# heitorrapela/HalluciDet

Measured on AMD Instinct MI355X. Metric: images/sec train_hallucidet (640x512, batch 8/GPU), higher is better.
Workload: dtype f16; 1 GPU; train_hallucidet.py fasterrcnn LLVIP batch=8 fp16 on 1xMI355X (BASELINE configs[1]); U-Net resnet34 fwd+bwd, 3 frozen Faster R-CNN R50-FPN passes @300x300 (one batched evaluation of 24 images: trunk, RPN, RoI heads, NMS for all three; the RGB / IR passes' LOSS VALUES, which the reference computes and discards, are not evaluated), loss scaling, value clip 0.5, Adam; global_batch=8, image=1x512x640 IR + 3x512x640 RGB, batch_per_gpu=8, parallelism=dp1

## Files before the change

### hallucidet_amd/_abi.py

```python
import ctypes as C
import os

_HERE = os.path.dirname(os.path.abspath(__file__))
LIB_PATH = os.environ.get("HD_HIP_LIB") or os.path.join(_HERE, "lib", "libhallucidet_hip.so")

ABI_VERSION = 6

HD_ACT_NONE, HD_ACT_RELU, HD_ACT_SIGMOID = 0, 1, 2
HD_OUT_NHWC_F16, HD_OUT_NCHW_F32, HD_OUT_NHWC_F32 = 0, 1, 2

c_i32 = C.c_int32
c_i64 = C.c_int64
c_f = C.c_float
c_d = C.c_double
vp = C.c_void_p


class HipLibraryMissing(RuntimeError):
    pass


class HipCallError(RuntimeError):
    pass


class ConvArgs(C.Structure):
    _fields_ = [
        ("x", vp), ("x2", vp), ("w", vp), ("bias", vp), ("res", vp), ("mask", vp), ("y", vp), ("stats", vp),
        ("N", c_i32), ("Hsrc", c_i32), ("Wsrc", c_i32), ("Hin", c_i32), ("Win", c_i32),
        ("C1", c_i32), ("C2", c_i32), ("Ho", c_i32), ("Wo", c_i32), ("Cout", c_i32),
        ("KH", c_i32), ("KW", c_i32), ("stride", c_i32), ("pad", c_i32),
        ("up1", c_i32), ("in_dil", c_i32), ("act", c_i32), ("out_mode", c_i32),
        ("in_scale", vp), ("in_shift", vp), ("in_relu", c_i32), ("out_pool2", c_i32),
        ("bs_y", vp), ("bs_z", vp), ("bs_mean", vp), ("bs_invstd", vp), ("bs_gamma", vp), ("bs_beta", vp), ("bs_relu", c_i32), ("reserved1", c_i32),
        ("y2", vp),
    ]


class WprepDesc(C.Structure):
    _fields_ = [("w_oihw", C.c_void_p), ("w_fwd", C.c_void_p), ("w_dgrad", C.c_void_p)] + \
               [(n, C.c_int32) for n in ("Cout", "Cin", "KH", "KW", "Cin_pad", "Cout_pad")]


class WredDesc(C.Structure):
    _fields_ = [("slab", C.c_void_p), ("dw_oihw", C.c_void_p)] + \
               [(n, C.c_int32) for n in ("nsplit", "Cout_slab", "Cout", "KH", "KW", "Cin", "Cin_real", "accumulate")] + \
               [("scale", C.c_float)] + [(n, C.c_int32) for n in ("mode", "first_block", "reserved")]


class WgradArgs(C.Structure):
    _fields_ = [
        ("x", vp), ("x2", vp), ("dy", vp), ("slab", vp),
        ("N", c_i32), ("Hsrc", c_i32), ("Wsrc", c_i32), ("Hin", c_i32), ("Win", c_i32),
        ("C1", c_i32), ("C2", c_i32), ("Ho", c_i32), ("Wo", c_i32), ("Cout", c_i32),
        ("KH", c_i32), ("KW", c_i32), ("stride", c_i32), ("pad", c_i32), ("up1", c_i32),
        ("nsplit", c_i32),
        ("in_scale", vp), ("in_shift", vp), ("in_relu", c_i32), ("reserved0", c_i32),
        ("dw_oihw", vp), ("dw_scale", c_f), ("reserved1", c_i32),
    ]


PROTOTYPES = {
    "hd_abi_version": (C.c_int, []),
    "hd_last_error": (C.c_char_p, []),
    "hd_arch": (C.c_char_p, []),
    "hd_conv2d": (C.c_int, [C.POINTER(ConvArgs), vp]),
    "hd_conv2d_stats_rows": (C.c_int, [C.POINTER(ConvArgs)]),
    "hd_conv2d_pool2_ok": (C.c_int, [C.POINTER(ConvArgs)]),
    "hd_conv2d_bstat_ok": (C.c_int, [C.POINTER(ConvArgs)]),
    "hd_conv7x7s2_dgrad_thin": (C.c_int, [vp, vp, vp, vp] + [C.c_int] * 5 + [vp]),
    "hd_conv_tune_override": (C.c_int, [C.c_int] * 4),
    "hd_conv_tune_w8": (C.c_int, [C.c_int, C.c_int]),
    "hd_conv_nominal_batch": (C.c_int, [C.c_int]),
    "hd_gemm_w8_mode": (C.c_int, [C.c_int]),
    "hd_wgrad_w8_blocks": (C.c_int, [C.POINTER(WgradArgs)]),
    "hd_wgrad": (C.c_int, [C.POINTER(WgradArgs), vp]),
    "hd_wgrad_multi": (C.c_int, [C.POINTER(WgradArgs), C.c_int, vp]),
    "hd_wgrad_direct_ok": (C.c_int, [C.POINTER(WgradArgs)]),
    "hd_conv2d_wgrad": (C.c_int, [C.POINTER(ConvArgs), C.POINTER(WgradArgs), vp]),
    "hd_conv2d_multi": (C.c_int, [C.POINTER(ConvArgs), C.c_int, vp]),
    "hd_wgrad_tune_override": (C.c_int, [C.c_int]),
    "hd_wgrad_reduce": (C.c_int, [vp, vp] + [C.c_int] * 7 + [c_f, C.c_int, vp]),
    "hd_wgrad_reduce_plan": (C.c_int, [vp, C.c_int]),
    "hd_wgrad_reduce_multi": (C.c_int, [vp, C.c_int, C.c_int, vp]),
    "hd_weight_prep": (C.c_int, [vp, vp, vp, vp] + [C.c_int] * 6 + [vp]),
    "hd_weight_prep_multi": (C.c_int, [vp, C.c_int, C.c_int, vp]),
    "hd_colsum": (C.c_int, [vp, C.c_int, C.c_int, vp, vp, vp]),
    "hd_rowsum": (C.c_int, [vp, C.c_int, C.c_int, vp, C.c_int, vp]),
    "hd_bn_finalize": (C.c_int, [vp, C.c_int, C.c_int, c_d, vp, vp, vp, vp, c_f, c_f, vp, vp, vp, vp, vp]),
    "hd_bn_eval_scale_shift": (C.c_int, [vp, vp, vp, vp, c_f, C.c_int, vp, vp, vp]),
    "hd_bn_apply": (C.c_int, [vp, vp, vp, vp, vp, c_i64, C.c_int, C.c_int, vp]),
    "hd_bn_bwd_reduce": (C.c_int, [vp] * 8 + [C.c_int, c_i64, C.c_int, C.c_int, vp]),
    "hd_bn_bwd_apply": (C.c_int, [vp] * 8 + [C.c_int] + [vp] * 5 + [c_f, C.c_int, c_i64, C.c_int, C.c_int, vp]),
    "hd_maxpool3x3s2": (C.c_int, [vp, vp] + [C.c_int] * 6 + [vp]),
    "hd_maxpool3x3s2_bwd": (C.c_int, [vp, vp, vp] + [C.c_int] * 6 + [vp]),
    "hd_maxpool3x3s2_idx": (C.c_int, [vp, vp, vp] + [C.c_int] * 6 + [vp]),
    "hd_maxpool3x3s2_bwd_idx": (C.c_int, [vp, vp, vp] + [C.c_int] * 6 + [vp]),
    "hd_maxpool3x3s2_bwd_idx_add": (C.c_int, [vp, vp, vp, vp] + [C.c_int] * 6 + [vp]),
    "hd_concat_up_bwd": (C.c_int, [vp, vp, vp] + [C.c_int] * 5 + [vp]),
    "hd_subsample2": (C.c_int, [vp, vp] + [C.c_int] * 6 + [vp]),
    "hd_subsample2_bwd": (C.c_int, [vp, vp] + [C.c_int] * 7 + [vp]),
    "hd_nchw_to_nhwc_resize": (C.c_int, [vp, vp] + [C.c_int] * 7 + [vp]),
    "hd_nchw_to_nhwc_resize_strided": (C.c_int, [vp, c_i64, c_i64, vp] + [C.c_int] * 7 + [vp]),
    "hd_nchw_to_nhwc_resize_bwd": (C.c_int, [vp, vp] + [C.c_int] * 7 + [c_f, vp]),
    "hd_nhwc_to_nchw": (C.c_int, [vp, vp] + [C.c_int] * 5 + [vp]),
    "hd_upsample_add": (C.c_int, [vp, vp, vp] + [C.c_int] * 6 + [vp]),
    "hd_upsample_add_bwd": (C.c_int, [vp, vp] + [C.c_int] * 7 + [vp]),
    "hd_upsample2_bwd": (C.c_int, [vp, vp] + [C.c_int] * 7 + [vp]),
    "hd_add_f16": (C.c_int, [vp, vp, vp, c_i64, vp]),
    "hd_slice_channels": (C.c_int, [vp, vp, c_i64, C.c_int, C.c_int, C.c_int, C.c_int, vp]),
    "hd_sigmoid_bwd_nchw_to_nhwc": (C.c_int, [vp, vp, vp] + [C.c_int] * 5 + [c_f, vp]),
    "hd_relu_bwd": (C.c_int, [vp, vp, vp, c_i64, vp]),
    "hd_f32_to_f16": (C.c_int, [vp, vp, c_i64, c_f, vp]),
    "hd_f16_to_f32": (C.c_int, [vp, vp, c_i64, c_f, vp]),
    "hd_pad_cast_f32_f16": (C.c_int, [vp, vp, C.c_int64, C.c_int, C.c_int, C.c_int64, C.c_int64, vp]),
    "hd_pad_cast_f32_f16_multi": (C.c_int, [vp, vp, vp, vp, vp, vp, vp, C.c_int, vp]),
    "hd_channel_sum_f16": (C.c_int, [vp, c_i64, C.c_int, vp, C.c_int, vp]),
    "hd_scale_store": (C.c_int, [vp, vp, C.c_int, c_f, C.c_int, vp]),
    "hd_nms_sorted_batched": (C.c_int, [vp, vp, C.c_int, C.c_int, c_f, vp, vp, vp]),
    "hd_nms_sorted_batched_topk": (C.c_int, [vp, vp, C.c_int, C.c_int, c_f, vp, vp, C.c_int, vp]),
    "hd_roi_align": (C.c_int, [vp, vp, vp] + [C.c_int] * 7 + [c_f, C.c_int, vp]),
    "hd_roi_align_ml": (C.c_int, [vp, vp, vp, vp, C.c_int, vp, vp, vp] + [C.c_int] * 5 + [vp]),
    "hd_roi_align_ml_bwd": (C.c_int, [vp, vp, vp, vp, vp, vp, vp] + [C.c_int] * 6 + [vp]),
    "hd_roi_align_ml_bwd_gather": (C.c_int, [vp, vp, vp, vp, vp, vp, vp] + [C.c_int] * 7 + [vp]),
    "hd_roi_align_bwd": (C.c_int, [vp, vp, vp] + [C.c_int] * 7 + [c_f, C.c_int, vp]),
    "hd_box_iou": (C.c_int, [vp, C.c_int, vp, C.c_int, vp, vp]),
    "hd_box_iou_batched": (C.c_int, [vp, C.c_int, vp, C.c_int, C.c_int, C.c_int, vp, vp]),
    "hd_rpn_loss": (C.c_int, [vp, vp, vp, vp, vp, vp, C.c_int64, C.c_float, vp, C.c_float, vp, vp, vp]),
    "hd_rpn_loss_bwd": (C.c_int, [vp, vp, vp, vp, vp, vp, C.c_int64, C.c_float, vp, vp, vp, C.c_float, vp, vp, vp]),
    "hd_retinanet_loss": (C.c_int, [vp] * 6 + [C.c_int] * 4 + [C.c_float] * 3 + [vp, vp, vp, vp, vp]),
    "hd_retinanet_loss_bwd": (C.c_int, [vp] * 6 + [C.c_int] * 4 + [C.c_float] * 3 + [vp] * 7),
    "hd_sigmoid_focal_loss": (C.c_int, [vp, vp, C.c_int64, C.c_float, C.c_float, vp, vp, vp]),
    "hd_groupnorm8_relu": (C.c_int, [vp] * 5 + [C.c_int] * 3 + [C.c_float, C.c_int, vp]),
    "hd_groupnorm8_relu_bwd": (C.c_int, [vp] * 6 + [C.c_int] * 4 + [vp]),
    "hd_groupnorm8_param_grad": (C.c_int, [vp] * 6 + [C.c_int] * 4 + [C.c_float, C.c_int, vp]),
    "hd_fcos_match": (C.c_int, [vp] * 3 + [C.c_int] * 5 + [C.c_float, vp, vp]),
    "hd_fcos_loss": (C.c_int, [vp] * 7 + [C.c_int] * 4 + [C.c_float] * 2 + [vp] * 4),
    "hd_fcos_loss_bwd": (C.c_int, [vp] * 7 + [C.c_int] * 4 + [C.c_float] * 2 + [vp] * 6),
    "hd_fastrcnn_loss": (C.c_int, [vp, vp, vp, vp, C.c_int, C.c_int, C.c_float, vp, vp, vp]),
    "hd_fastrcnn_loss_bwd": (C.c_int, [vp, vp, vp, vp, C.c_int, C.c_int, C.c_float, vp, vp, vp, vp, vp]),
    "hd_fastrcnn_loss_masked": (C.c_int, [vp, vp, vp, vp, C.c_int, C.c_int, C.c_float, vp, vp, vp, vp]),
    "hd_fastrcnn_loss_masked_bwd": (C.c_int, [vp, vp, vp, vp, C.c_int, C.c_int, C.c_float, vp, vp, vp, vp, vp, vp]),
    "hd_pixel_loss": (C.c_int, [vp, vp, vp] + [C.c_int] * 5 + [c_f, c_f, C.c_int] + [vp] * 6),
    "hd_map_match": (C.c_int, [vp] * 4 + [C.c_int] * 2 + [vp] * 3 + [C.c_int, vp, C.c_int] + [vp] * 9),
    "hd_map_accumulate": (C.c_int, [vp, vp, vp, c_i64, vp, vp, C.c_int, vp, vp, vp, vp]),
    "hd_sample_pos_neg": (C.c_int, [vp, vp, C.c_int, C.c_int, C.c_int, C.c_int, vp, vp, vp, vp]),
    "hd_roi_postprocess": (C.c_int, [vp, vp, vp, C.c_long, vp, C.c_int, C.c_int, C.c_int, vp] + [C.c_float] * 5 + [vp] * 4),
    "hd_roi_samples_padded": (C.c_int, [vp] * 7 + [C.c_int] * 4 + [vp] * 6),
    "hd_roi_samples_finish": (C.c_int, [vp, C.c_int, vp, vp, vp, vp, vp, C.c_int, C.c_int, vp, vp, vp, vp, vp]),
    "hd_roi_levels": (C.c_int, [vp, C.c_long, C.c_int, C.c_float, C.c_float, C.c_float, C.c_int, C.c_int, vp, vp]),
    "hd_batched_nms_pick": (C.c_int, [vp, vp, vp, vp, C.c_int, C.c_int, C.c_float, C.c_int, vp, vp, vp, vp, vp, vp, vp]),
    "hd_batched_nms_pick_segments": (C.c_int, [vp, vp, vp, C.c_int, C.c_int, vp, C.c_int, C.c_float, C.c_int, vp, vp, vp, vp, vp, vp, vp, vp, vp, vp]),
    "hd_rpn_decode_filter": (C.c_int, [vp, vp, vp, vp, C.c_int, C.c_int, C.c_int, C.c_float, C.c_float, C.c_float, C.c_float, C.c_float, vp, vp, vp, vp]),
    "hd_roi_decode_clip": (C.c_int, [vp, vp, C.c_long, C.c_int, C.c_int, vp, C.c_float, C.c_float, C.c_float, vp, vp]),
    "hd_topk_select_rows": (C.c_int, [vp, C.c_int, C.c_long, vp, C.c_int, C.c_int, vp, C.c_long, vp]),
    "hd_match_targets": (C.c_int, [vp, vp, vp, C.c_int, vp, C.c_int, C.c_int, C.c_int, C.c_float, C.c_float, C.c_int, vp, vp, vp, vp, vp, vp]),
    "hd_adam_step": (C.c_int, [vp, vp, vp, vp, c_i64] + [c_f] * 9 + [vp, vp]),
# ... 64 lines not shown
```

### hallucidet_amd/csrc/conv_dispatch.hip

```cpp
#include <stdlib.h>

#include "conv_params.h"

namespace {

int pick_bn(int Cout) { return Cout > 64 ? 128 : (Cout > 32 ? 64 : 32); }
int pick_bm(int M, int Cout) {
  int bn = pick_bn(Cout);
  int64_t blocks128 = (int64_t)hd_cdiv(M, 128) * hd_cdiv(Cout, bn);
  return (bn > 32 && blocks128 < 512) ? 64 : 128;
}

int fill_params(const hd_conv_args* a, ConvP& p) {
  HD_CHECK_ARG(a && a->x && a->w && a->y, "hd_conv2d: null pointer");
  HD_CHECK_ARG(a->C1 > 0 && a->C1 % 8 == 0 && a->C2 >= 0 && a->C2 % 8 == 0, "hd_conv2d: channel counts must be multiples of 8 (C1=%d C2=%d)", a->C1, a->C2);
  HD_CHECK_ARG((a->C2 == 0) == (a->x2 == nullptr), "hd_conv2d: x2/C2 mismatch");
  HD_CHECK_ARG(a->N > 0 && a->Ho > 0 && a->Wo > 0 && a->Cout > 0 && a->KH > 0 && a->KW > 0 && a->stride > 0, "hd_conv2d: bad extent");
  HD_CHECK_ARG(!(a->in_dil > 1 && (a->up1 || a->C2)), "hd_conv2d: in_dil excludes up1/x2");
  HD_CHECK_ARG(a->in_dil <= 2, "hd_conv2d: in_dil must be 1 or 2 (strides on the hot path)");
  HD_CHECK_ARG(a->C2 == 0 || (a->C1 % 32 == 0 && a->C2 % 32 == 0), "hd_conv2d: dual-source gather needs C1, C2 multiples of 32 (a K tile holds channels of one source)");
  HD_CHECK_ARG(!a->up1 || (a->Hin == 2 * a->Hsrc && a->Win == 2 * a->Wsrc), "hd_conv2d: up1 needs Hin=2*Hsrc");
  HD_CHECK_ARG((int64_t)a->N * a->Ho * a->Wo < (1ll << 31), "hd_conv2d: too many pixels");
  p.x = (const f16*)a->x;
  p.x2 = (const f16*)a->x2;
  p.w = (const f16*)a->w;
  p.bias = a->bias;
  p.res = (const f16*)a->res;
  p.mask = (const f16*)a->mask;
  p.y = a->y;
  p.stats = a->stats;
  p.N = a->N; p.Hsrc = a->Hsrc; p.Wsrc = a->Wsrc; p.Hin = a->Hin; p.Win = a->Win;
  p.C1 = a->C1; p.C2 = a->C2; p.Cin = a->C1 + a->C2;
  p.Ho = a->Ho; p.Wo = a->Wo; p.Cout = a->Cout; p.KH = a->KH; p.KW = a->KW;
  p.stride = a->stride; p.pad = a->pad; p.up1 = a->up1; p.in_dil = a->in_dil < 1 ? 1 : a->in_dil;
  p.act = a->act; p.out_mode = a->out_mode;
  HD_CHECK_ARG((a->in_scale == nullptr) == (a->in_shift == nullptr), "hd_conv2d: in_scale / in_shift must be given together");
  p.in_scale = a->in_scale; p.in_shift = a->in_shift; p.in_relu = a->in_relu;
  p.pool2 = a->out_pool2;
  p.y2 = a->y2;
  p.bs_y = (const f16*)a->bs_y; p.bs_z = (const f16*)a->bs_z;
  p.bs_mean = a->bs_mean; p.bs_invstd = a->bs_invstd; p.bs_gamma = a->bs_gamma; p.bs_beta = a->bs_beta; p.bs_relu = a->bs_relu;
  HD_CHECK_ARG(!p.bs_y || (p.stats && p.bs_mean && p.bs_invstd && !a->mask && a->act == HD_ACT_NONE && a->out_mode == HD_OUT_NHWC_F16 && !a->bias),
               "hd_conv2d: bs_* (BatchNorm backward sums) need stats, bs_mean, bs_invstd and exclude mask / act / bias / non-f16 output");
  HD_CHECK_ARG(p.out_mode >= HD_OUT_NHWC_F16 && p.out_mode <= HD_OUT_NHWC_F32, "hd_conv2d: out_mode %d", p.out_mode);
  p.M = a->N * a->Ho * a->Wo;
  p.cin8 = p.Cin / 8;
  p.nchunks = a->KH * a->KW * p.cin8;
  p.nk = 0;
  p.Ktot = a->KH * a->KW * p.Cin;
  p.prio = 0;
  p.par = p.ph = p.pw = p.Hc = p.Wc = p.t0h = p.t0w = 0;
  p.gm = p.gn = 0;
  p.tgroup = 1;
  p.inv_cin8 = 1.0f / (float)p.cin8;
  p.inv_kw = 1.0f / (float)a->KW;
  int64_t xb = (int64_t)a->N * a->Hsrc * a->Wsrc * a->C1 * 2;
  int64_t x2b = a->x2 ? (int64_t)a->N * a->Hin * a->Win * a->C2 * 2 : 0;
  int64_t wb = (int64_t)a->Cout * p.Ktot * 2;
  HD_CHECK_ARG(xb < 0xFFFFFFF0ll && x2b < 0xFFFFFFF0ll && wb < 0xFFFFFFF0ll, "hd_conv2d: tensor larger than 4 GiB (buffer addressing)");
  p.xbytes = (unsigned)xb; p.x2bytes = (unsigned)x2b; p.wbytes = (unsigned)wb;
  return HD_OK;
}

int env_int(const char* name, int dflt) {
  const char* v = getenv(name);
  return v ? atoi(v) : dflt;
}

}

static bool g_small_ok = true;

bool use_small(const ConvP& p) {
  static const int on = env_int("HD_CONV_SMALL", 1);
  return on && g_small_ok && hd_conv_small_eligible(p);
}

bool use_c64(const ConvP& p) {
  static const int on = env_int("HD_CONV_C64", 1);
  return on && g_small_ok && hd_conv_c64_eligible(p);
}

bool use_stem(const ConvP& p) {
  static const int on = env_int("HD_CONV_STEM", 1);
  return on && g_small_ok && hd_conv_stem_eligible(p);
}

bool use_c32(const ConvP& p) {
  static const int on = env_int("HD_CONV_C32", 1);
  return on && g_small_ok && !p.stats && hd_conv_c32to128_eligible(p);
}

bool use_cat(const ConvP& p) {
  static const int on = env_int("HD_CONV_CAT", 1);
  return on && g_small_ok && hd_conv_cat128to32_eligible(p);
}

static int g_gemm8_mode = -1;
extern "C" int hd_gemm_w8_mode(int mode) {
  HD_CHECK_ARG(mode == -1 || mode == 0 || mode == 128 || mode == 1128, "hd_gemm_w8_mode: mode in {-1, 0, 128, 1128}");
  g_gemm8_mode = mode;
  return HD_OK;
}
bool hd_gemm_w8_eligible(const ConvP& p);
void hd_gemm_w8_launch(ConvP& p, int tile, hipStream_t s);
static int choose_gemm8(const ConvP& p) {
  static const int on = env_int("HD_GEMM8", 1);
  if (!on || g_gemm8_mode == 0 || !g_small_ok || !hd_gemm_w8_eligible(p)) return 0;
  if (g_gemm8_mode > 0) return g_gemm8_mode;
  if (p.res || p.M < 2048 || p.Cout < 512 || p.Ktot < 512) return 0;
  const int64_t t128 = (int64_t)hd_cdiv(p.M, 256) * hd_cdiv(p.Cout, 128), t1128 = (int64_t)hd_cdiv(p.M, 128) * hd_cdiv(p.Cout, 128);
  if (t128 >= 160 && t128 <= 256) return 128;
  if (t1128 >= 200) return 1128;
  return 0;
}

static int g_ov_bm = -1, g_ov_bn = -1, g_ov_bk = -1, g_ov_deep = -1;
extern "C" int hd_conv_tune_override(int bm, int bn, int bk, int deep) {
  HD_CHECK_ARG((bm == -1 || bm == 64 || bm == 128) && (bn == -1 || bn == 32 || bn == 64 || bn == 128) && (bk == -1 || bk == 32 || bk == 64) &&
               deep >= -1 && deep <= 1, "hd_conv_tune_override: bm in {64,128}, bn in {32,64,128}, bk in {32,64}, deep in {0,1} or -1");
  g_ov_bm = bm; g_ov_bn = bn; g_ov_bk = bk; g_ov_deep = deep;
  g_small_ok = (bm == -1 && bn == -1 && bk == -1 && deep == -1);
  return HD_OK;
}

#ifdef HD_CONV_TRACE
static unsigned long long* g_trace = nullptr;
extern "C" int hd_conv_trace_buffer(void* buf) {
  g_trace = (unsigned long long*)buf;
  return HD_OK;
}
#endif

static int g_nominal_batch = 0;
extern "C" int hd_conv_nominal_batch(int n) {
  HD_CHECK_ARG(n >= 0 && n <= 4096, "hd_conv_nominal_batch: n in [0, 4096]");
  g_nominal_batch = n;
  return HD_OK;
}

static int choose_p8(const ConvP& p, bool allow_m160 = true) {
  static const int on = env_int("HD_CONV_P8", 1);
  if (!on || !hd_conv_p8_eligible(p)) return -1;
  if (p.Cout < 128 && !p.x2) return -1;
  static const int th[4] = {32, 16, 32, 16}, bn[4] = {128, 128, 64, 64};
  static const int ts = env_int("HD_W8_TS", 1);
  static const double step_ss[4] = {1270., 790., 800., 540.}, step_ts[4] = {1270., 790., 860., 450.}, fixed[4] = {11500., 8000., 9000., 7000.};
  double step[4];
  for (int c = 0; c < 4; ++c) step[c] = ((ts >= 2 && c >= 1) || (ts == 1 && c == 3)) ? step_ts[c] : step_ss[c];
  const int nk = p.nchunks / 8;
  int best = -1;
  double best_t = 1e30;
  static const int nominal = env_int("HD_CONV_NOMINAL_BATCH", 0);
  const int nominal_batch = g_nominal_batch > 0 ? g_nominal_batch : (nominal > 0 ? nominal : p.N);
  for (int c = 0; c < 4; ++c) {
    if (bn[c] == 128 && p.Cout <= 64) continue;
    const int64_t tm = (int64_t)nominal_batch * hd_cdiv(p.Ho, th[c]) * hd_cdiv(p.Wo, 8);
    const double eff = (double)((int64_t)nominal_batch * p.Ho * p.Wo) / (double)(tm * th[c] * 8);
    if (eff < 0.7) continue;
    const int64_t blocks = tm * hd_cdiv(p.Cout, bn[c]);
    const double t = (double)hd_cdiv(blocks, 256) * (fixed[c] + nk * step[c])   ;
    if (t < best_t) {
      best_t = t;
      best = c;
    }
  }
  best = ((ts >= 2 && best >= 1) || (ts == 1 && best == 3)) ? best + 4 : best;
  static const int m160_on = env_int("HD_CONV_M160", 1);
  static const double m160_fixed[2] = {(double)env_int("HD_M160_FIXED", 9000), (double)env_int("HD_M320_FIXED", 10500)};
  static const double m160_step[2] = {(double)env_int("HD_M160_STEP", 460), (double)env_int("HD_M320_STEP", 790)};
  if (m160_on && allow_m160 && hd_conv_m160_eligible(p)) {
    if (best < 0) {
      const int64_t b64 = (int64_t)hd_cdiv((int64_t)nominal_batch * p.Ho * p.Wo, 64) * hd_cdiv(p.Cout, 64);
      best_t = (double)hd_cdiv(b64, 512) * (4000. + nk * 900.);
    }
    static const double m96_fixed[2] = {(double)env_int("HD_M96_FIXED", 6600), (double)env_int("HD_M96_FIXED2", 11000)};
    static const double m96_step[2] = {(double)env_int("HD_M96_STEP", 350), (double)env_int("HD_M96_STEP2", 420)};
    static const int m96_on = env_int("HD_CONV_M96", 1);
    for (int v = 0; v < 3; ++v) {
      if (v == 2 && (!m96_on || p.x2)) continue;
      const int th_ = v == 1 ? 8 : 4, tw_ = v == 2 ? 24 : 40;
      const int64_t tm = (int64_t)nominal_batch * hd_cdiv(p.Ho, th_) * hd_cdiv(p.Wo, tw_);
      const int64_t blocks = tm * hd_cdiv(p.Cout, 64);
      double t;
      if (v == 2) {
        const int pair = blocks > 256;
        t = (double)(pair ? hd_cdiv(blocks, 512) : 1) * (m96_fixed[pair] + nk * m96_step[pair]);
      } else {
        t = (double)hd_cdiv(blocks, 256) * (m160_fixed[v] + nk * m160_step[v]);
      }
      if (t < best_t) {
        best_t = t;
        best = 8 + v;
      }
    }
  }
  return best;
// ... 154 lines not shown
  if (ok) {
    mp.n = n;
    const bool launched = c0.use64 ? hd_conv_launch_bk64_multi(mp, c0.bm, c0.bn, c0.deep, (hipStream_t)stream)
                                   : hd_conv_launch_bk32_multi(mp, c0.bm, c0.bn, c0.deep, (hipStream_t)stream);
    if (launched) {
      HD_CHECK_LAUNCH();
      return HD_OK;
    }
  }
  static const int m96_multi_on = env_int("HD_CONV_M96_MULTI", 1);
  bool taken[HD_CONV_MULTI_MAX] = {};
  if (multi_on && m96_multi_on && n >= 2 && n <= HD_CONV_MULTI_MAX && g_small_ok && g_w8_cfg < 0) {
    static ConvMulti m96;
    m96.n = 0;
    for (int i = 0; i < n; ++i) {
      ConvP& p = m96.p[m96.n];
      int rc = fill_params(&args[i], p);
      if (rc) return rc;
      if (use_small(p) || use_c64(p) || use_stem(p) || use_c32(p) || use_cat(p) || choose_gemm8(p) || p.pool2 || p.x2) continue;
      if (choose_tile(p).p8cfg != 10) continue;
      HD_CHECK_ARG(!p.bs_y || bstat_kernel(p), "hd_conv2d_multi: bs_* on a problem whose kernel does not implement them");
#ifdef HD_CONV_TRACE
      p.trace = nullptr;
      p.trace_tid = 0;
#endif
      taken[i] = true;
      ++m96.n;
    }
    if (m96.n >= 2) {
      hd_conv_launch_m96_multi(m96, (hipStream_t)stream);
      HD_CHECK_LAUNCH();
    } else {
      for (int i = 0; i < n; ++i) taken[i] = false;
    }
  }
  for (int i = 0; i < n; ++i) {
    if (taken[i]) continue;
    int rc = hd_conv2d(&args[i], stream);
    if (rc) return rc;
  }
  return HD_OK;
}

extern "C" int hd_conv2d(const hd_conv_args* a, void* stream) {
  ConvP p;
  int rc = fill_params(a, p);
  if (rc) return rc;
  hipStream_t s = (hipStream_t)stream;
#ifdef HD_CONV_TRACE
  p.trace = g_trace;
  p.trace_tid = env_int("HD_TRACE_TID", 0);
#endif
  HD_CHECK_ARG(!p.bs_y || bstat_kernel(p), "hd_conv2d: bs_* (BatchNorm backward sums) are implemented by the 8-wave and the 64-channel 3x3 kernels only; "
                                           "ask hd_conv2d_bstat_ok first");
  HD_CHECK_ARG(!p.pool2 || pool2_kernel(p),
               "hd_conv2d: out_pool2 is implemented by the small-channel 3x3 kernel (all channels pooled), the 32 -> 128 channel kernel "
               "(64 pooled channels + y2) and the 8-wave 3x3 family (pooled channels a multiple of 128); ask hd_conv2d_pool2_ok first");
  if (use_small(p)) {
    hd_conv_launch_small(p, s);
    HD_CHECK_LAUNCH();
    return HD_OK;
  }
  if (use_c64(p)) {
    hd_conv_launch_c64(p, s);
    HD_CHECK_LAUNCH();
    return HD_OK;
  }
  if (use_stem(p)) {
    hd_conv_launch_stem(p, s);
    HD_CHECK_LAUNCH();
    return HD_OK;
  }
  if (use_c32(p)) {
    hd_conv_launch_c32to128(p, s);
    HD_CHECK_LAUNCH();
    return HD_OK;
  }
  if (use_cat(p)) {
    hd_conv_launch_cat128to32(p, s);
    HD_CHECK_LAUNCH();
    return HD_OK;
  }
  if (const int g8 = choose_gemm8(p)) {
    hd_gemm_w8_launch(p, g8, s);
    HD_CHECK_LAUNCH();
    return HD_OK;
  }
  HD_CHECK_ARG(!p.in_scale, "hd_conv2d: consumer-side BatchNorm (in_scale / in_shift) is implemented by the small-channel 3x3 kernel only "
                            "(3x3 / stride 1 / pad 1, one source, C1 in {8,16,32}, Cout in {16,32} or a <= 16-channel fp32 head)");
  static const int par_on = env_int("HD_CONV_PARITY", 1);
  const bool par = par_on && p.in_dil == 2 && !p.stats && p.stride == 1 && (p.cin8 % 4) == 0 && p.out_mode == HD_OUT_NHWC_F16 && g_small_ok &&
                   g_w8_cfg < 0;
  const int M_full = p.M;
  if (par) p.M = p.N * ((p.Ho + 1) / 2) * ((p.Wo + 1) / 2);
  const TileChoice c = choose_tile(p);
  static const int w8_prio = env_int("HD_W8_PRIO", 0);
  p.prio = w8_prio;
  const int bm = c.bm, bn = c.bn;
  const bool use64 = c.use64, deep = c.deep;
  if (par && c.p8cfg < 0 && (c.use64 ? (p.cin8 % 8) == 0 : true)) {
    p.par = 1;
  } else {
    p.M = M_full;
  }
  if (c.p8cfg >= 8) {
    hd_conv_launch_m160(p, c.p8cfg == 9 ? 8 : 4, c.p8cfg == 10 ? 24 : 40, s);
  } else if (c.p8cfg >= 0) {
    hd_conv_launch_p8(p, c.p8cfg, s);
  } else if (use64) hd_conv_launch_bk64(p, bm, bn, deep, s);
  else hd_conv_launch_bk32(p, bm, bn, deep, s);
  HD_CHECK_LAUNCH();
  return HD_OK;
}
```

### include/hallucidet_hip.h

```cpp
#ifndef HALLUCIDET_HIP_H
#define HALLUCIDET_HIP_H

#include <stdint.h>

#ifdef __cplusplus
extern "C" {
#endif

#define HD_OK 0
#define HD_E_ARG (-1)
#define HD_E_LAUNCH (-2)
#define HD_E_UNSUPPORTED (-3)

#define HD_ACT_NONE 0
#define HD_ACT_RELU 1
#define HD_ACT_SIGMOID 2

#define HD_OUT_NHWC_F16 0
#define HD_OUT_NCHW_F32 1
#define HD_OUT_NHWC_F32 2

int hd_abi_version(void);
const char* hd_last_error(void);
const char* hd_arch(void);

typedef struct hd_conv_args {
  const void* x;
  const void* x2;
  const void* w;
  const float* bias;
  const void* res;
  const void* mask;
  void* y;
  float* stats;
  int32_t N, Hsrc, Wsrc;
  int32_t Hin, Win;
  int32_t C1, C2;
  int32_t Ho, Wo, Cout;
  int32_t KH, KW, stride, pad;
  int32_t up1, in_dil;
  int32_t act, out_mode;
  const float* in_scale;
  const float* in_shift;
  int32_t in_relu;
  int32_t out_pool2;
  const void* bs_y;
  const void* bs_z;
  const float* bs_mean;
  const float* bs_invstd;
  const float* bs_gamma;
  const float* bs_beta;
  int32_t bs_relu, reserved1;
  void* y2;
} hd_conv_args;

int hd_conv2d(const hd_conv_args* a, void* stream);
int hd_conv2d_bstat_ok(const hd_conv_args* a);
int hd_conv2d_pool2_ok(const hd_conv_args* a);
int hd_conv2d_stats_rows(const hd_conv_args* a);
int hd_conv7x7s2_dgrad_thin(const void* dy, const void* mask_z, const void* w16, void* dx, int N, int Hl, int Wl, int H, int W, void* stream);
int hd_conv_tune_override(int bm, int bn, int bk, int deep);
int hd_conv_tune_w8(int cfg, int nslices);
int hd_conv_nominal_batch(int n);
int hd_gemm_w8_mode(int mode);

typedef struct hd_wgrad_args {
  const void* x;
  const void* x2;
  const void* dy;
  float* slab;
  int32_t N, Hsrc, Wsrc, Hin, Win, C1, C2, Ho, Wo, Cout;
  int32_t KH, KW, stride, pad, up1;
  int32_t nsplit;
  const float* in_scale;
  const float* in_shift;
  int32_t in_relu, reserved0;
  float* dw_oihw;
  float dw_scale;
  int32_t reserved1;
} hd_wgrad_args;
int hd_wgrad(const hd_wgrad_args* a, void* stream);
int hd_wgrad_direct_ok(const hd_wgrad_args* a);
#define HD_WGRAD_MULTI_MAX 24
int hd_wgrad_multi(const hd_wgrad_args* args, int n, void* stream);
int hd_wgrad_w8_blocks(const hd_wgrad_args* a);
int hd_wgrad_tune_override(int tm);
int hd_conv2d_multi(const hd_conv_args* args, int n, void* stream);

int hd_conv2d_wgrad(const hd_conv_args* dgrad, const hd_wgrad_args* wgrad, void* stream);

int hd_wgrad_reduce(const float* slab, float* dw_oihw, int nsplit, int Cout_slab, int Cout, int KH, int KW,
                    int Cin, int Cin_real, float scale, int accumulate, void* stream);

#define HD_WRED_MAX 16
typedef struct hd_wred_desc {
  const float* slab;
  float* dw_oihw;
  int32_t nsplit, Cout_slab, Cout, KH, KW, Cin, Cin_real, accumulate;
  float scale;
  int32_t mode, first_block, reserved;
} hd_wred_desc;
int hd_wgrad_reduce_plan(hd_wred_desc* table_host, int n);
int hd_wgrad_reduce_multi(const hd_wred_desc* table_host, int n, int total_blocks, void* stream);

typedef struct hd_wprep_desc {
  const float* w_oihw;
  void* w_fwd;
  void* w_dgrad;
  int32_t Cout, Cin, KH, KW, Cin_pad, Cout_pad;
} hd_wprep_desc;

int hd_weight_prep(const float* w_oihw, const float* out_scale , void* w_fwd ,
                   void* w_dgrad , int Cout, int Cin, int KH, int KW,
                   int Cin_pad, int Cout_pad, void* stream);
int hd_weight_prep_multi(const hd_wprep_desc* table_dev, int n_layers, int blocks_per_layer, void* stream);

int hd_colsum(const float* in, int rows, int W, float* out, float* ws, void* stream);
int hd_rowsum(const float* in, int rows, int W, float* out, int out_rows, void* stream);
int hd_bn_finalize(const float* part, int rows, int C, double count, const float* gamma, const float* beta,
                   float* running_mean, float* running_var, float momentum, float eps, float* mean, float* invstd,
                   float* scale, float* shift, void* stream);
int hd_bn_eval_scale_shift(const float* gamma, const float* beta, const float* running_mean, const float* running_var,
                           float eps, int C, float* scale, float* shift, void* stream);
int hd_bn_apply(const void* y, const void* res, const float* scale, const float* shift, void* z, int64_t n, int C,
                int relu, void* stream);
int hd_bn_bwd_reduce(const void* dz, const void* z, const void* y, const float* mean, const float* invstd,
                     const float* gamma, const float* beta, float* part, int rows, int64_t npix, int C, int relu, void* stream);
int hd_bn_bwd_apply(const void* dz, const void* z, const void* y, const float* mean, const float* invstd,
                    const float* gamma, const float* beta, const float* part, int rows, float* coef_ws, void* dy, void* dres,
                    float* dgamma, float* dbeta, float gscale, int accumulate, int64_t npix, int C, int relu, void* stream);

int hd_maxpool3x3s2(const void* x, void* y, int N, int H, int W, int C, int Ho, int Wo, void* stream);
int hd_maxpool3x3s2_bwd(const void* x, const void* dy, void* dx, int N, int H, int W, int C, int Ho, int Wo, void* stream);
int hd_maxpool3x3s2_idx(const void* x, void* y, void* idx_u8, int N, int H, int W, int C, int Ho, int Wo, void* stream);
int hd_maxpool3x3s2_bwd_idx(const void* idx_u8, const void* dy, void* dx, int N, int H, int W, int C, int Ho, int Wo, void* stream);
int hd_maxpool3x3s2_bwd_idx_add(const void* idx_u8, const void* dy, const void* add, void* dx, int N, int H, int W, int C, int Ho, int Wo,
                                void* stream);
int hd_subsample2(const void* x, void* y, int N, int H, int W, int C, int Ho, int Wo, void* stream);
int hd_subsample2_bwd(const void* dy, void* dx, int N, int H, int W, int C, int Ho, int Wo, int accumulate, void* stream);
int hd_nchw_to_nhwc_resize(const float* x, void* y, int N, int Cr, int H, int W, int Ho, int Wo, int Cp, void* stream);
int hd_nchw_to_nhwc_resize_strided(const float* x, int64_t nstride, int64_t cstride, void* y, int N, int Cr, int H, int W, int Ho,
                                   int Wo, int Cp, void* stream);
int hd_nchw_to_nhwc_resize_bwd(const void* dy, float* dx, int N, int Cr, int H, int W, int Ho, int Wo, int Cp,
                               float gscale, void* stream);
int hd_nhwc_to_nchw(const void* x, float* y, int N, int Cr, int H, int W, int Cp, void* stream);
int hd_upsample_add(const void* a, const void* b, void* y, int N, int H, int W, int C, int Hb, int Wb, void* stream);
int hd_upsample_add_bwd(const void* dy, void* db, int N, int H, int W, int C, int Hb, int Wb, int accumulate, void* stream);
// ... 185 lines not shown
```

Baseline: 819.8 images/s.

## Add persistent producer-consumer GEMM kernel for large 1x1 convolutions

Adds a persistent, warp-specialized GEMM kernel. Four producer waves stream weight and activation tiles into a multi-stage LDS ring using buffer-load-to-LDS with counted waits, while four consumer waves run MFMA and a fused bias/residual/ReLU/mask epilogue. Tiles are distributed per XCD, and the grid is capped at the CU count. It is enabled by default for the shapes that previously chose the w8 GEMM tiles (128 maps to BM=256, 1128 maps to BM=128), aiming to hide global-load latency and cut launch/tail overhead. The risks are lower MFMA occupancy with only half the waves computing, and a fixed requirement that K be a multiple of 64.

```diff
diff --git a/hallucidet_amd/_abi.py b/hallucidet_amd/_abi.py
--- a/hallucidet_amd/_abi.py
+++ b/hallucidet_amd/_abi.py
@@ -73,6 +73,7 @@
     "hd_conv_tune_w8": (C.c_int, [C.c_int, C.c_int]),
     "hd_conv_nominal_batch": (C.c_int, [C.c_int]),
     "hd_gemm_w8_mode": (C.c_int, [C.c_int]),
+    "hd_gemm_pc_mode": (C.c_int, [C.c_int, C.c_int]),
     "hd_wgrad_w8_blocks": (C.c_int, [C.POINTER(WgradArgs)]),
     "hd_wgrad": (C.c_int, [C.POINTER(WgradArgs), vp]),
     "hd_wgrad_multi": (C.c_int, [C.POINTER(WgradArgs), C.c_int, vp]),
diff --git a/hallucidet_amd/csrc/conv_dispatch.hip b/hallucidet_amd/csrc/conv_dispatch.hip
--- a/hallucidet_amd/csrc/conv_dispatch.hip
+++ b/hallucidet_amd/csrc/conv_dispatch.hip
@@ -104,15 +104,28 @@
 }
 bool hd_gemm_w8_eligible(const ConvP& p);
 void hd_gemm_w8_launch(ConvP& p, int tile, hipStream_t s);
+static int g_gemm_pc_mode = -1, g_gemm_pc_blocks = 0;
+extern "C" int hd_gemm_pc_mode(int tile, int max_blocks) {
+  HD_CHECK_ARG((tile == -1 || tile == 0 || tile == 128 || tile == 256) && max_blocks >= 0, "hd_gemm_pc_mode: tile in {-1, 0, 128, 256}, max_blocks >= 0");
+  g_gemm_pc_mode = tile;
+  g_gemm_pc_blocks = max_blocks;
+  return HD_OK;
+}
+void hd_gemm_pc_launch(ConvP& p, int tile, int max_blocks, hipStream_t s);
 static int choose_gemm8(const ConvP& p) {
   static const int on = env_int("HD_GEMM8", 1);
-  if (!on || g_gemm8_mode == 0 || !g_small_ok || !hd_gemm_w8_eligible(p)) return 0;
+  static const int pc_on = env_int("HD_GEMM_PC", 1);
+  if (!g_small_ok || !hd_gemm_w8_eligible(p)) return 0;
+  if (g_gemm_pc_mode > 0) return 2000 + g_gemm_pc_mode;
+  if (!on || g_gemm8_mode == 0) return 0;
   if (g_gemm8_mode > 0) return g_gemm8_mode;
+  int t = 0;
   if (p.res || p.M < 2048 || p.Cout < 512 || p.Ktot < 512) return 0;
   const int64_t t128 = (int64_t)hd_cdiv(p.M, 256) * hd_cdiv(p.Cout, 128), t1128 = (int64_t)hd_cdiv(p.M, 128) * hd_cdiv(p.Cout, 128);
-  if (t128 >= 160 && t128 <= 256) return 128;
-  if (t1128 >= 200) return 1128;
-  return 0;
+  if (t128 >= 160 && t128 <= 256) t = 128;
+  else if (t1128 >= 200) t = 1128;
+  if (t && pc_on && g_gemm_pc_mode != 0) return t == 128 ? 2256 : 2128;
+  return t;
 }
 
 static int g_ov_bm = -1, g_ov_bn = -1, g_ov_bk = -1, g_ov_deep = -1;
@@ -433,7 +446,8 @@
     return HD_OK;
   }
   if (const int g8 = choose_gemm8(p)) {
-    hd_gemm_w8_launch(p, g8, s);
+    if (g8 > 2000) hd_gemm_pc_launch(p, g8 - 2000, g_gemm_pc_blocks, s);
+    else hd_gemm_w8_launch(p, g8, s);
     HD_CHECK_LAUNCH();
     return HD_OK;
   }
diff --git a/hallucidet_amd/csrc/gemm_pc.hip b/hallucidet_amd/csrc/gemm_pc.hip
--- /dev/null
+++ b/hallucidet_amd/csrc/gemm_pc.hip
@@ -0,0 +1,252 @@
+#include "hd_common.h"
+#include "conv_params.h"
+
+namespace {
+
+constexpr int GK = 64;
+constexpr int GROW = 64;
+constexpr unsigned GOOB = 0xFFFFFFF0u;
+constexpr int EPI = 32 * GROW;
+
+typedef __attribute__((address_space(3))) void lds_void_pc;
+
+__device__ __forceinline__ void pdma16(__amdgpu_buffer_rsrc_t r, f16* lds_dst, unsigned voff) {
+  __builtin_amdgcn_raw_ptr_buffer_load_lds(r, (lds_void_pc*)lds_dst, 16, voff, 0, 0, 0);
+}
+
+template <int L>
+__device__ __forceinline__ void wait_steps(int n) {
+  if (n >= 2) asm volatile("s_waitcnt vmcnt(%0)" ::"n"(2 * L) : "memory");
+  else if (n == 1) asm volatile("s_waitcnt vmcnt(%0)" ::"n"(L) : "memory");
+  else asm volatile("s_waitcnt vmcnt(0)" ::: "memory");
+}
+
+template <int BM, int NSTAGE>
+struct PC {
+  static constexpr int BN = 128;
+  static constexpr int NB = BM / 64;
+  static constexpr int STAGE = (BM + BN) * GROW;
+  static constexpr int W_PASS = BN / 32, X_PASS = BM / 32;
+  static constexpr int L = W_PASS + X_PASS;
+  static constexpr int AHEAD = NSTAGE - 1;
+  static constexpr int LDS_HALVES = NSTAGE * STAGE + 4 * EPI;
+  static_assert(LDS_HALVES * 2 <= 160 * 1024, "LDS");
+  static_assert(AHEAD >= 2 && AHEAD <= 3 && (AHEAD - 1) * L <= 63, "counted wait");
+};
+
+template <int BM, int NSTAGE>
+__global__ __launch_bounds__(512, 1) void gemm_pc_kernel(ConvP p) {
+  using G = PC<BM, NSTAGE>;
+  constexpr int BN = G::BN, NB = G::NB, STAGE = G::STAGE, W_PASS = G::W_PASS, X_PASS = G::X_PASS, L = G::L, AHEAD = G::AHEAD;
+  __shared__ __attribute__((aligned(1024))) f16 lds[G::LDS_HALVES];
+
+  const int tid = threadIdx.x, lane = tid & 63;
+  const int wave = __builtin_amdgcn_readfirstlane(tid >> 6);
+  const bool consumer = wave < 4;
+  const int K = p.Ktot, nk = K / GK;
+
+  const int ntile = p.gm * p.gn, nwg = gridDim.x, bid = blockIdx.x;
+  const int xcd = bid & 7, q = bid >> 3;
+  const int first = xcd * (ntile >> 3) + (xcd < (ntile & 7) ? xcd : (ntile & 7));
+  const int count = (ntile >> 3) + (xcd < (ntile & 7) ? 1 : 0);
+  const int nblk = (nwg >> 3) + (xcd < (nwg & 7) ? 1 : 0);
+  const int ntb = q < count ? (count - q + nblk - 1) / nblk : 0;
+  const int S = ntb * nk;
+  auto tile_at = [&](int ord, int& tm, int& tn) { hd_conv_tile_of(p, first + q + ord * nblk, tm, tn); };
+
+  if (!consumer) {
+    const int ptid = tid - 256, pw = wave - 4;
+    const __amdgpu_buffer_rsrc_t rx = __builtin_amdgcn_make_buffer_rsrc(const_cast<f16*>(p.x), 0, p.xbytes, 0x00020000);
+    const __amdgpu_buffer_rsrc_t rw = __builtin_amdgcn_make_buffer_rsrc(const_cast<f16*>(p.w), 0, p.wbytes, 0x00020000);
+    const int j = (ptid & 7) ^ ((ptid >> 4) & 7);
+    unsigned wbase[W_PASS], xbase[X_PASS];
+    bool wok[W_PASS], xok[X_PASS];
+    auto bases = [&](int ord) {
+      int tm, tn;
+      tile_at(ord, tm, tn);
+#pragma unroll
+      for (int i = 0; i < W_PASS; ++i) {
+        const int row = tn * BN + i * 32 + (ptid >> 3);
+        wok[i] = row < p.Cout;
+        wbase[i] = (unsigned)(wok[i] ? row : 0) * (unsigned)K * 2u + (unsigned)j * 16u;
+      }
+#pragma unroll
+      for (int i = 0; i < X_PASS; ++i) {
+        const int row = tm * BM + i * 32 + (ptid >> 3);
+        xok[i] = row < p.M;
+        xbase[i] = (unsigned)(xok[i] ? row : 0) * (unsigned)K * 2u + (unsigned)j * 16u;
+      }
+    };
+    int it = 0, ikt = 0, wr = 0;
+    auto issue = [&]() {
+      f16* sw = lds + wr * STAGE + pw * (8 * GROW);
+      f16* sx = sw + BN * GROW;
+      const unsigned ko = (unsigned)ikt * (GK * 2);
+#pragma unroll
+      for (int i = 0; i < W_PASS; ++i) pdma16(rw, sw + i * (32 * GROW), wok[i] ? wbase[i] + ko : GOOB);
+#pragma unroll
+      for (int i = 0; i < X_PASS; ++i) pdma16(rx, sx + i * (32 * GROW), xok[i] ? xbase[i] + ko : GOOB);
+      wr = wr + 1 == NSTAGE ? 0 : wr + 1;
+      if (++ikt == nk) {
+        ikt = 0;
+        if (++it < ntb) bases(it);
+      }
+    };
+    if (S > 0) bases(0);
+    for (int t = 0; t < AHEAD && t < S; ++t) issue();
+    wait_steps<L>((S - 1 < AHEAD - 1 ? S - 1 : AHEAD - 1));
+    __builtin_amdgcn_s_barrier();
+    for (int t = 0; t < S; ++t) {
+      if (t + AHEAD < S) issue();
+      wait_steps<L>((S - 1 < t + AHEAD ? S - 1 : t + AHEAD) - (t + 1));
+      __builtin_amdgcn_s_barrier();
+    }
+    asm volatile("s_waitcnt vmcnt(0)" ::: "memory");
+    return;
+  }
+
+  const int wn = wave & 1, wm = wave >> 1;
+  const int frow = lane & 31, fh = lane >> 5, swz = (frow >> 1) & 7;
+  f32x16 acc[2][NB];
+  auto zero = [&]() {
+#pragma unroll
+    for (int a = 0; a < 2; ++a)
+#pragma unroll
+      for (int b = 0; b < NB; ++b)
+#pragma unroll
+        for (int r = 0; r < 16; ++r) acc[a][b][r] = 0.f;
+  };
+  zero();
+  f16x8 wf[2][2], xf[2][NB];
+  auto frag = [&](int stage, int ks, int buf) {
+    const f16* sw = lds + stage * STAGE;
+    const f16* sx = sw + BN * GROW;
+    const int slot = ((ks * 2 + fh) ^ swz) * 8;
+#pragma unroll
+    for (int a = 0; a < 2; ++a) wf[buf][a] = *reinterpret_cast<const f16x8*>(sw + (wn * 64 + a * 32 + frow) * GROW + slot);
+#pragma unroll
+    for (int b = 0; b < NB; ++b) xf[buf][b] = *reinterpret_cast<const f16x8*>(sx + (wm * (BM / 2) + b * 32 + frow) * GROW + slot);
+  };
+
+  f16* const ep = lds + NSTAGE * STAGE + wave * EPI;
+  f16* __restrict__ yp = reinterpret_cast<f16*>(p.y);
+  const f16* __restrict__ maskp = p.mask;
+  const f16* __restrict__ resp = p.res;
+  const float* __restrict__ biasp = p.bias;
+  const bool relu = p.act == HD_ACT_RELU;
+  const int N = p.Cout, M = p.M;
+  const int er = lane >> 3, eq = lane & 7;
+  auto epilogue = [&](int ord) {
+    int tm, tn;
+    tile_at(ord, tm, tn);
+    const int c0 = tn * BN + wn * 64;
+    const int cq = c0 + 8 * eq;
+#pragma unroll
+    for (int b = 0; b < NB; ++b) {
+      const int rb = tm * BM + wm * (BM / 2) + b * 32;
+      if (resp) {
+        f16x8 rv[4];
+#pragma unroll
+        for (int i = 0; i < 4; ++i) {
+          const int m = rb + er + 8 * i;
+          rv[i] = f16x8{};
+          if (m < M && cq < N) rv[i] = *reinterpret_cast<const f16x8*>(resp + (size_t)m * N + cq);
+        }
+#pragma unroll
+        for (int i = 0; i < 4; ++i) *reinterpret_cast<f16x8*>(ep + (er + 8 * i) * GROW + ((eq ^ er) * 8)) = rv[i];
+        asm volatile("s_waitcnt lgkmcnt(0)" ::: "memory");
+      }
+#pragma unroll
+      for (int a = 0; a < 2; ++a)
+#pragma unroll
+        for (int g = 0; g < 4; ++g) {
+          f16* pp = ep + frow * GROW + (((4 * a + g) ^ (frow & 7)) * 8) + 4 * fh;
+          const int c = c0 + 32 * a + 8 * g + 4 * fh;
+          f32x4 bv = {0.f, 0.f, 0.f, 0.f};
+          if (biasp && c < N) bv = *reinterpret_cast<const f32x4*>(biasp + c);
+          f16x4 rv = {(f16)0.f, (f16)0.f, (f16)0.f, (f16)0.f};
+          if (resp) rv = *reinterpret_cast<const f16x4*>(pp);
+          f16x4 o;
+#pragma unroll
+          for (int i = 0; i < 4; ++i) {
+            float v = acc[a][b][4 * g + i];
+            if (resp) v += (float)rv[i];
+            v += bv[i];
+            if (relu) v = fmaxf(v, 0.f);
+            o[i] = (f16)v;
+          }
+          *reinterpret_cast<f16x4*>(pp) = o;
+        }
+      asm volatile("s_waitcnt lgkmcnt(0)" ::: "memory");
+#pragma unroll
+      for (int i = 0; i < 4; ++i) {
+        const int m = rb + er + 8 * i;
+        f16x8 ov = *reinterpret_cast<const f16x8*>(ep + (er + 8 * i) * GROW + ((eq ^ er) * 8));
+        if (m < M && cq < N) {
+          const size_t off = (size_t)m * N + cq;
+          if (maskp) {
+            const f16x8 mv = *reinterpret_cast<const f16x8*>(maskp + off);
+#pragma unroll
+            for (int k = 0; k < 8; ++k) ov[k] = ((float)mv[k] > 0.f) ? ov[k] : (f16)0.f;
+          }
+          *reinterpret_cast<f16x8*>(yp + off) = ov;
+        }
+      }
+      asm volatile("s_waitcnt lgkmcnt(0)" ::: "memory");
+    }
+  };
+
+  __builtin_amdgcn_s_barrier();
+  __builtin_amdgcn_s_setprio(1);
+  int rd = 0, kt = 0, ord = 0;
+  for (int t = 0; t < S; ++t) {
+    __builtin_amdgcn_sched_barrier(0);
+    frag(rd, 0, 0);
+    frag(rd, 1, 1);
+#pragma unroll
+    for (int ks = 0; ks < GK / 16; ++ks) {
+      __builtin_amdgcn_sched_barrier(0);
+#pragma unroll
+      for (int a = 0; a < 2; ++a)
+#pragma unroll
+        for (int b = 0; b < NB; ++b) acc[a][b] = __builtin_amdgcn_mfma_f32_32x32x16_f16(wf[ks & 1][a], xf[ks & 1][b], acc[a][b], 0, 0, 0);
+      __builtin_amdgcn_sched_barrier(0);
+      if (ks + 2 < GK / 16) frag(rd, ks + 2, ks & 1);
+    }
+    __builtin_amdgcn_sched_barrier(0);
+    asm volatile("s_waitcnt lgkmcnt(0)" ::: "memory");
+    __builtin_amdgcn_s_barrier();
+    __builtin_amdgcn_sched_barrier(0);
+    rd = rd + 1 == NSTAGE ? 0 : rd + 1;
+    if (++kt == nk) {
+      kt = 0;
+      __builtin_amdgcn_s_setprio(0);
+      epilogue(ord++);
+      zero();
+      __builtin_amdgcn_s_setprio(1);
+    }
+  }
+  __builtin_amdgcn_s_setprio(0);
+}
+
+int g_cus = 0;
+
+}
+
+void hd_gemm_pc_launch(ConvP& p, int tile, int max_blocks, hipStream_t s) {
+  if (g_cus <= 0) {
+    int dev = 0, n = 0;
+    if (hipGetDevice(&dev) != hipSuccess || hipDeviceGetAttribute(&n, hipDeviceAttributeMultiprocessorCount, dev) != hipSuccess || n <= 0) n = 256;
+    g_cus = n;
+  }
+  const int bm = tile == 256 ? 256 : 128;
+  p.gm = hd_cdiv(p.M, bm);
+  p.gn = hd_cdiv(p.Cout, 128);
+  p.tgroup = hd_conv_tile_order(p);
+  int grid = p.gm * p.gn;
+  if (grid > g_cus) grid = g_cus;
+  if (max_blocks > 0 && grid > max_blocks) grid = max_blocks;
+  if (grid < 8 && grid < p.gm * p.gn) grid = p.gm * p.gn < 8 ? p.gm * p.gn : 8;
+  if (tile == 256) hipLaunchKernelGGL((gemm_pc_kernel<256, 3>), dim3(grid), dim3(512), 0, s, p);
+  else hipLaunchKernelGGL((gemm_pc_kernel<128, 4>), dim3(grid), dim3(512), 0, s, p);
+}
diff --git a/include/hallucidet_hip.h b/include/hallucidet_hip.h
--- a/include/hallucidet_hip.h
+++ b/include/hallucidet_hip.h
@@ -63,6 +63,7 @@
 int hd_conv_tune_w8(int cfg, int nslices);
 int hd_conv_nominal_batch(int n);
 int hd_gemm_w8_mode(int mode);
+int hd_gemm_pc_mode(int tile, int max_blocks);
 
 typedef struct hd_wgrad_args {
   const void* x;
```

Measured after the change: 827.2 images/s (median of 6 runs). About the same (+0.9%).
